# anshulahuja98/antidote

Hardware: AMD Instinct MI355X
Metric: materialized ops/sec + VC compares/sec (1/2/4/8 GPU), % of HBM roofline (higher is better)
Workload: dtype u64; 1 GPU; cfg2 counter_pn materialize: 10M keys x 64 ops/key, 8-DC clocks, random snapshot VCs; keys_per_gpu=10000000, keys_total=10000000, ops_per_key=64, n_dcs=8, r_jitter=U[-2000,2000], partitioning=vnode p = key mod 64, gpu = p mod G; no collective, parallelism=dp1

## Files before the change

antidote_amd/csrc/mat_counter_dense.hip:

```cpp
#include <atomic>
#include <cstdlib>
#include <vector>

#include "counter_scan.hpp"

namespace agn {
namespace {

constexpr uint32_t QL_S = 1024, QL_STRIDE = 32;

inline uint32_t counter_order(uint64_t n_req, uint32_t bulk) {
    return order_or(n_req < (1ull << 20) ? 1u : bulk);
}
constexpr uint32_t BULK_CHUNK = 64;
constexpr uint32_t BULK_CHUNK4 = 64;
constexpr bool Q2_FOUR_DEFAULT = true;
constexpr uint32_t BULK_CHUNK8 = 64;
constexpr uint64_t NARROW_WIDE_DIV = 1024;
constexpr bool EFF16_DEFAULT = true;
constexpr uint64_t EFF16_ESC_DIV = 1024;

struct DenseArgs {
    uint64_t n_req;
    uint64_t n_entries;
// ... 690 lines not shown
                                         uint32_t *__restrict__ o_count,
                                         uint32_t *__restrict__ o_flags,
                                         uint32_t *__restrict__ o_err,
                                         uint64_t *__restrict__ o_mask) {
    const int lane = lane_id();
    const uint64_t i = k.i;
    if (k.corrupt) {
        if (lane == 0) {
            o_flags[i] = AGN_F_ERR_CORRUPTED;
            o_err[i] = 0xffffffffu;
        }
        return;
    }
    if (lane < 4) {
        u64x2 v;
        v.x = r.ct_ign ? 0ull : s.ctA;
        v.y = r.ct_ign ? 0ull : s.ctB;
        reinterpret_cast<u64x2 *>(o_lastct + i * 8u)[lane] = v;
    }
    if (lane == 0) {
        o_value[i] = r.value;
        o_hole[i] = r.hole;
        o_count[i] = r.cnt;
        o_err[i] = r.err;
        o_flags[i] = r.fl;
        if (r.wm) o_mask[i] = r.mo;
    }
}

typedef long long i64x2 __attribute__((ext_vector_type(2)));
typedef unsigned int u32x2 __attribute__((ext_vector_type(2)));

__device__ __forceinline__ void q2_store2(uint64_t i0, const Q2Acc &s0, const Q2Acc &s1,
                                          const Q2Out &r0, const Q2Out &r1,
                                          int64_t *__restrict__ o_value,
                                          int64_t *__restrict__ o_hole,
                                          uint64_t *__restrict__ o_lastct,
                                          uint32_t *__restrict__ o_count,
                                          uint32_t *__restrict__ o_flags,
                                          uint32_t *__restrict__ o_err,
                                          uint64_t *__restrict__ o_mask) {
    const int lane = lane_id();
    if (lane < 8) {
        const bool hi = lane >= 4;
        const bool ign = hi ? r1.ct_ign : r0.ct_ign;
        u64x2 v;
        v.x = ign ? 0ull : (hi ? s1.ctA : s0.ctA);
        v.y = ign ? 0ull : (hi ? s1.ctB : s0.ctB);
        reinterpret_cast<u64x2 *>(o_lastct + i0 * 8u)[lane] = v;
    }
    if (lane == 0) {
        *reinterpret_cast<i64x2 *>(o_value + i0) = i64x2{r0.value, r1.value};
        *reinterpret_cast<i64x2 *>(o_hole + i0) = i64x2{r0.hole, r1.hole};
        *reinterpret_cast<u32x2 *>(o_count + i0) = u32x2{r0.cnt, r1.cnt};
        *reinterpret_cast<u32x2 *>(o_err + i0) = u32x2{r0.err, r1.err};
        *reinterpret_cast<u32x2 *>(o_flags + i0) = u32x2{r0.fl, r1.fl};
        if (r0.wm && r1.wm) {
            *reinterpret_cast<u64x2 *>(o_mask + i0) = u64x2{r0.mo, r1.mo};
        } else {
            if (r0.wm) o_mask[i0] = r0.mo;
            if (r1.wm) o_mask[i0 + 1u] = r1.mo;
        }
    }
}

struct Q2Params {
    DenseArgs a;
    MaskArgs mk;
    const uint64_t *keys, *key_off, *key_len;
    const uint8_t *key_type;
    const uint32_t *key_id0;
    const uint64_t *oc;
    const uint32_t *op_id;
    const int64_t *eff;
    const uint64_t *log_txid, *R, *sct;
    const uint8_t *sct_ignore;
    const uint64_t *req_txid;
    const int64_t *base_value;
    int64_t *o_value, *o_hole;
    uint64_t *o_lastct;
    uint32_t *o_count, *o_flags, *o_err, *list, *list_n;
};

template <class T>
__device__ __forceinline__ DenseArgs dense_of(const T &x) {
    return DenseArgs{x.n_req, x.n_entries, x.req_type, x.xcd, x.pair, x.qnt, x.hints, x.ql_cap};
}
template <class T>
__device__ __forceinline__ MaskArgs mask_of(const T &x) {
    return MaskArgs{x.key_mask, x.oc_mask, x.R_mask, x.sct_mask, x.o_mask};
}

__device__ __forceinline__ uint32_t put_lane(uint32_t v, int g, uint32_t old) {
    return lane_id() == g ? v : old;
}

struct Q2PackParams {
    DenseArgs a;
    MaskArgs mk;
    const void *args[20];
    const uint32_t *rows;
    const uint64_t *base;
    const uint8_t *ok;
};
static_assert(offsetof(Q2PackParams, rows) == offsetof(Q2Params, list),
              "Q2PackParams follows k_counter_quad2's parameter list");

__device__ __forceinline__ u32x4 q2_pack_thr(const Q2Key &k, const Q2Pack &p, bool &noR) {
    noR = ballot(k.rA < p.bq.x || k.rB < p.bq.y) != 0ull;
    const uint64_t dA = k.rA - p.bq.x, dB = k.rB - p.bq.y;
    const uint32_t tA = (dA >> 32) ? 0xFFFFFFFFu : (uint32_t)dA;
    const uint32_t tB = (dB >> 32) ? 0xFFFFFFFFu : (uint32_t)dB;
    u32x4 t;
    t.x = __builtin_amdgcn_update_dpp(0u, tA, 0x88, 0xF, 0xF, false);
    t.y = __builtin_amdgcn_update_dpp(0u, tB, 0x88, 0xF, 0xF, false);
    t.z = __builtin_amdgcn_update_dpp(0u, tA, 0xDD, 0xF, 0xF, false);
    t.w = __builtin_amdgcn_update_dpp(0u, tB, 0xDD, 0xF, 0xF, false);
    return t;
}

__device__ __forceinline__ void q2_pack_ct(const Q2Pack &p, u32x4 mx, Q2Acc &s) {
#pragma unroll
    for (int x = 2; x < AGN_WAVE; x <<= 1) {
        const uint32_t a = (uint32_t)__shfl_xor((int)mx.x, x, AGN_WAVE);
        const uint32_t b = (uint32_t)__shfl_xor((int)mx.y, x, AGN_WAVE);
        const uint32_t c = (uint32_t)__shfl_xor((int)mx.z, x, AGN_WAVE);
        const uint32_t d = (uint32_t)__shfl_xor((int)mx.w, x, AGN_WAVE);
        mx.x = a > mx.x ? a : mx.x;
        mx.y = b > mx.y ? b : mx.y;
        mx.z = c > mx.z ? c : mx.z;
        mx.w = d > mx.w ? d : mx.w;
    }
    const uint32_t g0 = __builtin_amdgcn_update_dpp(0u, mx.x, 0x50, 0xF, 0xF, false);
    const uint32_t g1 = __builtin_amdgcn_update_dpp(0u, mx.y, 0x50, 0xF, 0xF, false);
    const uint32_t g2 = __builtin_amdgcn_update_dpp(0u, mx.z, 0x50, 0xF, 0xF, false);
    const uint32_t g3 = __builtin_amdgcn_update_dpp(0u, mx.w, 0x50, 0xF, 0xF, false);
    const bool hi = (lane_id() & 1) != 0;
    s.ctA = s.cnt ? p.bq.x + (uint64_t)(hi ? g2 : g0) : 0ull;
    s.ctB = s.cnt ? p.bq.y + (uint64_t)(hi ? g3 : g1) : 0ull;
}

__device__ __forceinline__ void q2_serve_oc(const DenseArgs &a, uint64_t i) {
    const MaskArgs mk{};
    const auto &p = kparams<Q2Params>();
    const Q2Key k = q2_prologue<false, false>(a, mk, i, p.keys, p.key_off, p.key_len, p.key_type,
                                              p.key_id0, p.R, p.sct, p.sct_ignore, p.req_txid);
    Q2Acc s;
    s.ctA = k.eA;
    s.ctB = k.eB;
    if (a.n_entries != 0 && !k.corrupt)
        scan_key_q8<false, true, false, false>(p.oc, p.eff, nullptr, 0ull, k.off, k.n, a.n_entries,
                                               k.rA, k.rB, k.sA, k.sB, s.ctA, s.ctB, s.sum, s.cnt,
                                               s.first_excl, s.first_err, k.noR);
    const auto &pe = kparams<Q2Params>();
    q2_epilogue<false>(k, s, a.hints, pe.op_id, pe.base_value, pe.o_value, pe.o_hole, pe.o_lastct,
                       pe.o_count, pe.o_flags, pe.o_err, nullptr);
}

template <bool ANY_WARM, bool MSK, bool Q2_EFF, bool Q2_STORE, bool PACK = false>
__global__ __launch_bounds__(64, (ANY_WARM && !MSK) ? 6 : 1) void k_counter_quad2(
    DenseArgs a, MaskArgs mk, const uint64_t *__restrict__ keys,
    const uint64_t *__restrict__ key_off, const uint64_t *__restrict__ key_len,
    const uint8_t *__restrict__ key_type, const uint32_t *__restrict__ key_id0,
    const uint64_t *__restrict__ oc, const uint32_t *__restrict__ op_id,
    const int64_t *__restrict__ eff, const uint64_t *__restrict__ log_txid,
    const uint64_t *__restrict__ R, const uint64_t *__restrict__ sct,
    const uint8_t *__restrict__ sct_ignore, const uint64_t *__restrict__ req_txid,
    const int64_t *__restrict__ base_value, int64_t *__restrict__ o_value,
    int64_t *__restrict__ o_hole, uint64_t *__restrict__ o_lastct,
    uint32_t *__restrict__ o_count, uint32_t *__restrict__ o_flags,
    uint32_t *__restrict__ o_err, const uint32_t *__restrict__ pack_rows,
    const uint64_t *__restrict__ pack_base, const uint8_t *__restrict__ pack_ok) {
    static_assert(!PACK || (!ANY_WARM && !MSK && Q2_EFF && Q2_STORE),
                  "packed rows: the cold dense form only");
    const uint32_t blk = block_order(a.xcd, blockIdx.x, gridDim.x);
    const uint64_t i0 = uniform_u64((uint64_t)blk * 2u);
    if (i0 >= a.n_req) return;
    const bool two = i0 + 1u < a.n_req;
    const uint64_t i1 = two ? i0 + 1u : i0;
    Q2Pack pk0{}, pk1{};
    const Q2Key k0 = q2_prologue<ANY_WARM, MSK, PACK>(a, mk, i0, keys, key_off, key_len, key_type,
                                                      key_id0, R, sct, sct_ignore, req_txid,
                                                      pack_base, pack_ok, &pk0);
    const Q2Key k1 = q2_prologue<ANY_WARM, MSK, PACK>(a, mk, i1, keys, key_off, key_len, key_type,
                                                      key_id0, R, sct, sct_ignore, req_txid,
                                                      pack_base, pack_ok, &pk1);
    Q2Acc s0, s1;
    s0.ctA = k0.eA;
    s0.ctB = k0.eB;
    s1.ctA = k1.eA;
    s1.ctB = k1.eB;
    if constexpr (Q2_EFF || Q2_STORE) {
        const bool one = k0.n <= (uint64_t)AGN_WAVE && k1.n <= (uint64_t)AGN_WAVE;
        if (a.n_entries != 0 && one && (!MSK || (k0.uni && k1.uni)) &&
            (!PACK || (pk0.ok & pk1.ok) != 0u)) {
            const bool d0 = !k0.corrupt, d1 = !k1.corrupt;
            uint64_t in0 = 0, in1 = 0;
            int64_t ev0 = 0, ev1 = 0;
            u32x4 m0 = {0u, 0u, 0u, 0u}, m1 = {0u, 0u, 0u, 0u};
            if constexpr (PACK) {
                const uint32_t *const rows = kparams<Q2PackParams>().rows;
                const P8Rows c0 = p8_load_rows<true>(rows, k0.off, 0, a.n_entries);
                const P8Rows c1 = p8_load_rows<true>(rows, k1.off, 0, a.n_entries);
                const int64_t *const l_eff = (const int64_t *)kparams<Q2Params>().eff;
                const uint64_t *const l_R = (const uint64_t *)kparams<Q2Params>().R;
                __builtin_amdgcn_sched_barrier(0);
                bool nr0, nr1;
                const u32x4 th0 = q2_pack_thr(k0, pk0, nr0), th1 = q2_pack_thr(k1, pk1, nr1);
                Q2Acc t0 = s0, t1 = s1;
                in0 = p8_verdict(c0, 0, k0.n, th0, nr0, m0, t0.cnt, t0.first_excl);
                in0 = d0 ? in0 : 0ull;
                if (d0) s0 = t0;
                ev0 = q8_load_eff(l_eff, k0.off, 0, in0, reinterpret_cast<const int64_t *>(l_R + k0.i * 8u));
                in1 = p8_verdict(c1, 0, k1.n, th1, nr1, m1, t1.cnt, t1.first_excl);
                in1 = d1 ? in1 : 0ull;
                if (d1) s1 = t1;
                ev1 = q8_load_eff(l_eff, k1.off, 0, in1, reinterpret_cast<const int64_t *>(l_R + k1.i * 8u));
                __builtin_amdgcn_sched_barrier(0);
            } else if constexpr (Q2_EFF) {
                const Q8Rows c0 = q8_load_rows<true>(oc, k0.off, 0, a.n_entries);
                const Q8Rows c1 = q8_load_rows<true>(oc, k1.off, 0, a.n_entries);
                __builtin_amdgcn_sched_barrier(0);
                Q2Acc t0 = s0, t1 = s1;
                in0 = q2_verdict<ANY_WARM>(k0, c0, log_txid, a.n_entries, t0);
                in0 = d0 ? in0 : 0ull;
                if (d0) s0 = t0;
                ev0 = q8_load_eff(eff, k0.off, 0, in0, reinterpret_cast<const int64_t *>(R + k0.i * 8u));
                in1 = q2_verdict<ANY_WARM>(k1, c1, log_txid, a.n_entries, t1);
                in1 = d1 ? in1 : 0ull;
                if (d1) s1 = t1;
                ev1 = q8_load_eff(eff, k1.off, 0, in1, reinterpret_cast<const int64_t *>(R + k1.i * 8u));
                __builtin_amdgcn_sched_barrier(0);
            } else {
                const Q8Chunk c0 = q8_load<true, false>(oc, eff, k0.off, 0, a.n_entries);
                const Q8Chunk c1 = q8_load<true, false>(oc, eff, k1.off, 0, a.n_entries);
                __builtin_amdgcn_sched_barrier(0);
                if (d0) q2_fold<ANY_WARM>(k0, c0, 0, log_txid, a.n_entries, s0);
                if (d1) q2_fold<ANY_WARM>(k1, c1, 0, log_txid, a.n_entries, s1);
            }
            const auto &pr = kparams<Q2Params>();
            const uint32_t *const l_op_id = pr.op_id;
            const int64_t *const l_base = pr.base_value;
            int64_t *const l_value = pr.o_value, *const l_hole = pr.o_hole;
            uint64_t *const l_lastct = pr.o_lastct;
            uint32_t *const l_count = pr.o_count, *const l_flags = pr.o_flags, *const l_err = pr.o_err;
            if constexpr (PACK) {
                q2_pack_ct(pk0, m0, s0);
                q2_pack_ct(pk1, m1, s1);
            } else {
                q2_ctfold<MSK>(k0, s0);
                q2_ctfold<MSK>(k1, s1);
            }
            if constexpr (Q2_EFF) {
                __builtin_amdgcn_sched_barrier(0);
                q8_fold_eff(in0, ev0, 0, s0.sum, s0.first_err);
                q8_fold_eff(in1, ev1, 0, s1.sum, s1.first_err);
                __builtin_amdgcn_sched_barrier(0);
            }
            Q2Out r0{}, r1{};
            if (d0) r0 = q2_result<MSK>(k0, s0, a.hints, l_op_id, l_base, mk.o_mask != nullptr);
            if (two && d1) r1 = q2_result<MSK>(k1, s1, a.hints, l_op_id, l_base, mk.o_mask != nullptr);
            if (Q2_STORE && two && d0 && d1) {
                q2_store2(i0, s0, s1, r0, r1, l_value, l_hole, l_lastct, l_count, l_flags, l_err, mk.o_mask);
            } else {
                q2_store(k0, s0, r0, l_value, l_hole, l_lastct, l_count, l_flags, l_err, mk.o_mask);
                if (two) q2_store(k1, s1, r1, l_value, l_hole, l_lastct, l_count, l_flags, l_err, mk.o_mask);
            }
            return;
        }
    }
    if constexpr (PACK) {
#pragma nounroll
        for (uint32_t h = 0; h < (two ? 2u : 1u); ++h) q2_serve_oc(a, i0 + h);
        return;
    }
    if (a.n_entries != 0) {
        const Q8Chunk c0 = q8_load<true, false>(oc, eff, k0.off, 0, a.n_entries);
        const Q8Chunk c1 = q8_load<true, false>(oc, eff, k1.off, 0, a.n_entries);
        __builtin_amdgcn_sched_barrier(0);
        const bool d0 = !k0.corrupt && (!MSK || k0.uni), d1 = !k1.corrupt && (!MSK || k1.uni);
        if (d0) q2_fold<ANY_WARM>(k0, c0, 0, log_txid, a.n_entries, s0);
        if (d1) q2_fold<ANY_WARM>(k1, c1, 0, log_txid, a.n_entries, s1);
        if (d0) q2_rest<ANY_WARM>(k0, oc, eff, log_txid, a.n_entries, s0);
        if (d1) q2_rest<ANY_WARM>(k1, oc, eff, log_txid, a.n_entries, s1);
        if constexpr (MSK) {
            if (!k0.corrupt && !k0.uni)
                q2_msk<ANY_WARM>(k0, oc, mk.oc_mask, eff, log_txid, a.n_entries, s0);
            if (!k1.corrupt && !k1.uni)
                q2_msk<ANY_WARM>(k1, oc, mk.oc_mask, eff, log_txid, a.n_entries, s1);
        }
    }
    if constexpr (Q2_EFF || Q2_STORE) {
        const auto &pe = kparams<Q2Params>();
        q2_epilogue<MSK>(k0, s0, a.hints, pe.op_id, pe.base_value, pe.o_value, pe.o_hole, pe.o_lastct,
                         pe.o_count, pe.o_flags, pe.o_err, mk.o_mask);
        if (two)
            q2_epilogue<MSK>(k1, s1, a.hints, pe.op_id, pe.base_value, pe.o_value, pe.o_hole,
                             pe.o_lastct, pe.o_count, pe.o_flags, pe.o_err, mk.o_mask);
        return;
    }
    q2_epilogue<MSK>(k0, s0, a.hints, op_id, base_value, o_value, o_hole, o_lastct, o_count, o_flags, o_err,
                     mk.o_mask);
    if (two)
        q2_epilogue<MSK>(k1, s1, a.hints, op_id, base_value, o_value, o_hole, o_lastct, o_count, o_flags,
                         o_err, mk.o_mask);
}

__global__ __launch_bounds__(64) void k_counter_pack4(Q2PackParams) {
    const DenseArgs a = dense_of(kparams<Q2Params>().a);
    const uint32_t blk = block_order(a.xcd, blockIdx.x, gridDim.x);
    const uint64_t i0 = uniform_u64((uint64_t)blk * 4u);
    if (i0 >= a.n_req) return;
    const int lane = lane_id();
    if (i0 + 3u < a.n_req) {
        const auto &pm = kparams<Q2Params>();
        const uint64_t *const key_off = pm.key_off, *const key_len = pm.key_len;
        const uint32_t *const key_id0 = pm.key_id0;
        const uint8_t *const key_type = pm.key_type;
        const uint64_t *const R = pm.R;
        const auto &pq = *(const __attribute__((address_space(4))) Q2PackParams *)&pm;
        const uint64_t *const pbase = pq.base;
        const uint8_t *const pok = pq.ok;
        const int64_t *const bvp = pm.base_value;
        const u64x4 offv = ldc_u64x4(key_off + i0);
        const u64x4 lenv = ldc_u64x4(key_len ? key_len + i0 : key_off + i0);
        const u32x4 idv = ldc_u32x4(key_id0 ? key_id0 + i0
                                            : reinterpret_cast<const uint32_t *>(key_off + i0));
        const uint8_t *const ktp = key_type ? key_type : reinterpret_cast<const uint8_t *>(key_off);
        uint64_t off[5], ln[4];
        uint32_t id0[4];
        off[4] = uniform_u64(ldc(key_len ? key_off + i0 : key_off + i0 + 4u));
        uint32_t ktw = __builtin_amdgcn_readfirstlane(ldc(reinterpret_cast<const uint32_t *>(ktp) + (i0 >> 2)));
        uint32_t okw = __builtin_amdgcn_readfirstlane(ldc(reinterpret_cast<const uint32_t *>(pok) + (i0 >> 2)));
        const uint64_t slot = i0 * 8u + (uint64_t)p4_slot(lane);
        const uint64_t rv = R[slot], bv = pbase[slot];
        const uint64_t bvl = *(bvp ? reinterpret_cast<const uint64_t *>(bvp) + (i0 + (uint64_t)(lane & 3))
                                   : R + slot);
        const uint64_t reqbase = bvp ? bvl : 0ull;
#pragma unroll
        for (int g = 0; g < 4; ++g) {
            off[g] = uniform_u64(offv[g]);
            ln[g] = uniform_u64(lenv[g]);
            id0[g] = (uint32_t)__builtin_amdgcn_readfirstlane(idv[g]);
        }
        asm volatile("" : "+s"(off[0]), "+s"(off[1]), "+s"(off[2]), "+s"(off[3]), "+s"(off[4]),
                          "+s"(ln[0]), "+s"(ln[1]), "+s"(ln[2]), "+s"(ln[3]), "+s"(id0[0]),
                          "+s"(id0[1]), "+s"(id0[2]), "+s"(id0[3]), "+s"(ktw), "+s"(okw));
        const bool has_len = key_len != nullptr, has_id0 = key_id0 != nullptr;
        const uint32_t want = key_type != nullptr ? (a.req_type & 0xffu) * 0x01010101u : ktw;
        uint32_t n[4];
        uint32_t bad = (okw ^ 0x01010101u) | (a.n_entries == 0 ? 1u : 0u);
#pragma unroll
        for (int g = 0; g < 4; ++g) {
            const uint64_t n64 = has_len ? ln[g] : off[g + 1] - off[g];
            n[g] = (uint32_t)n64;
            id0[g] = has_id0 ? id0[g] : AGN_ID0_NONE;
            const uint32_t kdiff = ((ktw ^ want) >> (8 * g)) & 0xffu;
            bad |= (n64 > (uint64_t)AGN_WAVE ? 1u : 0u) | (n64 != 0 ? kdiff : 0u);
        }
        if (bad == 0u) {
            const uint32_t *const rows = kparams<Q2PackParams>().rows;
            P8Rows c[4];
#pragma unroll
            for (int g = 0; g < 4; ++g) c[g] = p8_load_rows<true>(rows, off[g], 0, a.n_entries);
            const int64_t *const l_eff = kparams<Q2Params>().eff;
            __builtin_amdgcn_sched_barrier(0);
            const uint64_t below = ballot(rv < bv);
            const uint64_t dl = rv - bv;
            const uint32_t t = (dl >> 32) ? 0xFFFFFFFFu : (uint32_t)dl;
            uint32_t v_off_lo = 0, v_off_hi = 0, v_n = 0, v_id0 = 0, v_cnt = 0, v_fx = 0, v_fe = 0,
                     v_sum_lo = 0, v_sum_hi = 0;
            uint32_t cg = 0;
            const int kg = lane >> 4;
            u32x4 mx[4];
            uint64_t in[4];
            int64_t ev[4];
#pragma unroll
            for (int g = 0; g < 4; ++g) {
                const u32x4 th = p4_thr(t, g);
                const bool noR = ((below >> (16 * g)) & 0xFFFFull) != 0ull;
                uint32_t cnt = 0;
                int64_t fx = -1;
                mx[g] = u32x4{0u, 0u, 0u, 0u};
                in[g] = p8_verdict(c[g], 0, (uint64_t)n[g], th, noR, mx[g], cnt, fx);
                ev[g] = q8_load_eff(l_eff, off[g], 0, in[g],
                                    reinterpret_cast<const int64_t *>(R + (i0 + (uint64_t)g) * 8u));
                __builtin_amdgcn_sched_barrier(0);
                cg = kg == g ? cnt : cg;
                v_cnt = put_lane(cnt, g, v_cnt);
                v_fx = put_lane((uint32_t)fx, g, v_fx);
                v_off_lo = put_lane((uint32_t)off[g], g, v_off_lo);
                v_off_hi = put_lane((uint32_t)(off[g] >> 32), g, v_off_hi);
                v_n = put_lane(n[g], g, v_n);
                v_id0 = put_lane(id0[g], g, v_id0);
            }
            __builtin_amdgcn_sched_barrier(0);
            const auto &pr = kparams<Q2Params>();
            const uint32_t *const l_op_id = pr.op_id;
            int64_t *const l_value = pr.o_value, *const l_hole = pr.o_hole;
            uint64_t *const l_lastct = pr.o_lastct;
            uint32_t *const l_count = pr.o_count, *const l_flags = pr.o_flags, *const l_err = pr.o_err;
            const uint64_t v_off = ((uint64_t)v_off_hi << 32) | v_off_lo;
            const int32_t fx = (int32_t)v_fx;
            const uint32_t pos = fx >= 0 ? (uint32_t)fx : v_n - 1u;
            const bool need = lane < 4 && v_id0 == AGN_ID0_NONE && v_n != 0u;
            const uint32_t *const ip = need ? l_op_id + (v_off + (uint64_t)pos)
                                            : reinterpret_cast<const uint32_t *>(R + slot);
            const uint32_t opid = *ip;
            const uint32_t md = p4_maxfold(mx);
            const uint64_t ct = cg ? bv + (uint64_t)md : 0ull;
            __builtin_amdgcn_sched_barrier(0);
#pragma unroll
            for (int g = 0; g < 4; ++g) {
                int64_t sum = 0, fe = -1;
                q8_fold_eff(in[g], ev[g], 0, sum, fe);
                const uint64_t total = (uint64_t)wave_sum_dpp(sum);
                v_fe = put_lane((uint32_t)fe, g, v_fe);
                v_sum_lo = put_lane((uint32_t)total, g, v_sum_lo);
                v_sum_hi = put_lane((uint32_t)(total >> 32), g, v_sum_hi);
            }
            __builtin_amdgcn_sched_barrier(0);
            const uint64_t idh = v_id0 != AGN_ID0_NONE ? (uint64_t)v_id0 + (uint64_t)pos : (uint64_t)opid;
            const int64_t hid = v_n ? (int64_t)idh : 0;
            const int32_t fe = (int32_t)v_fe;
            uint32_t fl = v_cnt ? AGN_F_NEWSS : AGN_F_CT_IGNORE;
            fl |= fe >= 0 ? AGN_F_ERR_UNEXPECTED : 0u;
            if ((lane & 2) == 0) l_lastct[slot] = ct;
            if (lane < 4) {
                const uint64_t i = i0 + (uint64_t)lane;
                l_value[i] = (int64_t)(reqbase + (((uint64_t)v_sum_hi << 32) | v_sum_lo));
                l_hole[i] = fx >= 0 ? hid - 1 : hid;
                l_count[i] = v_cnt;
                l_err[i] = fe >= 0 ? (uint32_t)(v_off + (uint64_t)fe) : 0xffffffffu;
                l_flags[i] = fl;
            }
            return;
        }
    }
    const uint64_t left = a.n_req - i0;
    const uint32_t m = left < 4u ? (uint32_t)left : 4u;
#pragma nounroll
    for (uint32_t h = 0; h < m; ++h) q2_serve_oc(a, i0 + h);
}

struct Q2Pack8Params {
    DenseArgs a;
    MaskArgs mk;
    const void *args[20];
    const uint32_t *rows;
    const uint64_t *base;
    const uint8_t *ok;
    const uint16_t *rows16;
    const uint8_t *narrow;
    const int16_t *eff16;
};
static_assert(offsetof(Q2Pack8Params, rows) == offsetof(Q2PackParams, rows) &&
                  offsetof(Q2Pack8Params, base) == offsetof(Q2PackParams, base),
              "Q2Pack8Params extends Q2PackParams");

template <bool E16>
__global__ __launch_bounds__(64) void k_counter_pack8(Q2Pack8Params) {
    const DenseArgs a = dense_of(kparams<Q2Params>().a);
    const uint32_t blk = block_order(a.xcd, blockIdx.x, gridDim.x);
    const uint64_t i0 = uniform_u64((uint64_t)blk * 8u);
    if (i0 >= a.n_req) return;
    const int lane = lane_id();
    if (i0 + 7u < a.n_req) {
        const auto &pm = kparams<Q2Params>();
        const uint64_t *const key_off = pm.key_off, *const key_len = pm.key_len;
        const uint32_t *const key_id0 = pm.key_id0;
        const uint8_t *const key_type = pm.key_type;
        const uint64_t *const R = pm.R;
        const int64_t *const bvp = pm.base_value;
        const auto &pq = *(const __attribute__((address_space(4))) Q2Pack8Params *)&pm;
        const uint64_t *const pbase = pq.base;
        const uint8_t *const pnar = pq.narrow;
        const bool has_len = key_len != nullptr, has_id0 = key_id0 != nullptr;
        const uint32_t m8 = (uint32_t)lane & 7u;
        const uint64_t *const op = key_off + i0 + (uint64_t)((!has_len && lane >= 8) ? 8u : m8);
        const uint64_t v_off = *op;
        const uint64_t v_lr = *(has_len ? key_len + i0 + m8 : op);
        const uint32_t v_ir = *(has_id0 ? key_id0 + i0 + m8 : reinterpret_cast<const uint32_t *>(op));
        const uint8_t *const ktp = key_type ? key_type : reinterpret_cast<const uint8_t *>(key_off);
        uint32_t ktw0 = __builtin_amdgcn_readfirstlane(ldc(reinterpret_cast<const uint32_t *>(ktp) + (i0 >> 2)));
        uint32_t ktw1 = __builtin_amdgcn_readfirstlane(ldc(reinterpret_cast<const uint32_t *>(ktp) + (i0 >> 2) + 1u));
        uint32_t nw0 = __builtin_amdgcn_readfirstlane(ldc(reinterpret_cast<const uint32_t *>(pnar) + (i0 >> 2)));
        uint32_t nw1 = __builtin_amdgcn_readfirstlane(ldc(reinterpret_cast<const uint32_t *>(pnar) + (i0 >> 2) + 1u));
        const uint64_t slot = i0 * 8u + (uint64_t)lane;
        const uint64_t rv = R[slot], bv = pbase[slot];
        const uint64_t bvl = *(bvp ? reinterpret_cast<const uint64_t *>(bvp) + (i0 + m8) : R + slot);
        const uint64_t reqbase = bvp ? bvl : 0ull;
        const uint64_t v_nx =
            ((uint64_t)__builtin_amdgcn_update_dpp(0u, (uint32_t)(v_off >> 32), 0x101, 0xF, 0xF, false) << 32) |
            __builtin_amdgcn_update_dpp(0u, (uint32_t)v_off, 0x101, 0xF, 0xF, false);
        const uint64_t v_n64 = has_len ? v_lr : v_nx - v_off;
        const uint32_t v_n = (uint32_t)v_n64;
        const uint32_t v_id0 = has_id0 ? v_ir : AGN_ID0_NONE;
        const uint32_t kt = (((lane & 4) ? ktw1 : ktw0) >> (8u * ((uint32_t)lane & 3u))) & 0xffu;
        const uint32_t want = key_type != nullptr ? (a.req_type & 0xffu) : kt;
        const bool lbad = lane < 8 && (v_n64 > (uint64_t)AGN_WAVE || (v_n64 != 0 && kt != want));
        const bool bad = ballot(lbad) != 0ull || nw0 != 0x01010101u || nw1 != 0x01010101u ||
                         a.n_entries == 0;
        if (!bad) {
            const uint16_t *const rows16 = kparams<Q2Pack8Params>().rows16;
            u32x4 c[8];
#pragma unroll
            for (int g = 0; g < 8; ++g)
                c[g] = n8_load_rows<true>(rows16, n8_readlane_u64(v_off, g), a.n_entries);
            const int64_t *const l_eff = kparams<Q2Params>().eff;
            uint32_t e16[E16 ? 8 : 1];
            if constexpr (E16) {
                const int16_t *const eff16 = kparams<Q2Pack8Params>().eff16;
#pragma unroll
                for (int g = 0; g < 8; ++g)
                    e16[g] = n8_load_eff16(eff16, n8_readlane_u64(v_off, g), a.n_entries);
            }
            __builtin_amdgcn_sched_barrier(0);
            const uint64_t below = ballot(rv < bv);
            const uint64_t dl = rv - bv;
            const uint32_t tp = n8_thr_pack(dl > 0xFFFFull ? 0xFFFFu : (uint32_t)dl);
            uint32_t v_cnt = 0, v_fx = 0, v_fe = E16 ? 0xFFFFFFFFu : 0u, v_inc = 0;
            uint32_t cg = 0;
            const int kg = lane >> 3;
            int64_t ev[E16 ? 1 : 8];
#pragma unroll
            for (int g = 0; g < 8; ++g) {
                const uint32_t th0 = __builtin_amdgcn_readlane(tp, 8 * g);
                const uint32_t th1 = __builtin_amdgcn_readlane(tp, 8 * g + 2);
                const uint32_t th2 = __builtin_amdgcn_readlane(tp, 8 * g + 4);
                const uint32_t th3 = __builtin_amdgcn_readlane(tp, 8 * g + 6);
                const uint32_t noR = (uint32_t)(below >> (8 * g)) & 0xFFu;
                const uint32_t n_g = __builtin_amdgcn_readlane(v_n, g);
                const uint64_t off_g = n8_readlane_u64(v_off, g);
                const bool valid = (uint32_t)lane < n_g;
                const bool ex = (noR | n8_excl(c[g], th0, th1, th2, th3)) != 0u;
                const bool mine = valid & !ex;
                const uint64_t exm = ballot(valid & ex);
                const uint32_t cnt = (uint32_t)__builtin_popcountll(ballot(mine));
                const uint32_t fx = exm ? (uint32_t)__builtin_ctzll(exm) : 0xFFFFFFFFu;
                if constexpr (!E16)
                    ev[g] = n8_load_eff(l_eff, off_g, mine,
                                        reinterpret_cast<const int64_t *>(R + (i0 + (uint64_t)g) * 8u));
                c[g].x = mine ? c[g].x : 0u;
                c[g].y = mine ? c[g].y : 0u;
                c[g].z = mine ? c[g].z : 0u;
                c[g].w = mine ? c[g].w : 0u;
                v_inc |= mine ? (1u << g) : 0u;
                __builtin_amdgcn_sched_barrier(0);
                cg = kg == g ? cnt : cg;
                v_cnt = put_lane(cnt, g, v_cnt);
                v_fx = put_lane(fx, g, v_fx);
            }
            __builtin_amdgcn_sched_barrier(0);
            const auto &pr = kparams<Q2Params>();
            const uint32_t *const l_op_id = pr.op_id;
            int64_t *const l_value = pr.o_value, *const l_hole = pr.o_hole;
            uint64_t *const l_lastct = pr.o_lastct;
            uint32_t *const l_count = pr.o_count, *const l_flags = pr.o_flags, *const l_err = pr.o_err;
            const int32_t fx = (int32_t)v_fx;
            const uint32_t pos = fx >= 0 ? (uint32_t)fx : v_n - 1u;
            const bool need = lane < 8 && v_id0 == AGN_ID0_NONE && v_n != 0u;
            const uint32_t *const ip = need ? l_op_id + (v_off + (uint64_t)pos)
                                            : reinterpret_cast<const uint32_t *>(R + slot);
            uint32_t opid = 0;
            if (!E16 || ballot(need) != 0ull) opid = *ip;
            uint32_t v_esc = 0, ks32 = 0;
            if constexpr (E16) {
                uint32_t sm[8];
#pragma unroll
                for (int g = 0; g < 8; ++g) {
                    const bool mine = ((v_inc >> g) & 1u) != 0u;
                    const bool esc = mine && e16[g] == 0x8000u;
                    v_esc |= esc ? (1u << g) : 0u;
                    sm[g] = (mine && !esc) ? (uint32_t)(int32_t)(int16_t)e16[g] : 0u;
                }
                ks32 = n8_sumfold32(sm);
                __builtin_amdgcn_sched_barrier(0);
            }
            const uint32_t md = n8_maxfold(c);
            const uint64_t ct = cg ? bv + (uint64_t)md : 0ull;
            __builtin_amdgcn_sched_barrier(0);
            uint64_t total;
            if constexpr (E16) {
                total = (uint64_t)(int64_t)(int32_t)__shfl((int)ks32, 8 * (int)m8, AGN_WAVE);
                if (ballot(v_esc != 0u) != 0ull) {
#pragma nounroll
                    for (int g = 0; g < 8; ++g) {
                        const bool esc = ((v_esc >> g) & 1u) != 0u;
                        if (ballot(esc) == 0ull) continue;
                        const uint64_t off_g = n8_readlane_u64(v_off, g);
                        int64_t x = 0;
                        if (esc) x = l_eff[off_g + (uint64_t)lane];
                        const bool badv = esc && x == AGN_EFFECT_INVALID;
                        const uint64_t be = ballot(badv);
                        const uint64_t xs = (uint64_t)wave_sum_dpp(badv ? 0 : x);
                        v_fe = put_lane(be ? (uint32_t)__builtin_ctzll(be) : 0xFFFFFFFFu, g, v_fe);
                        total += lane == g ? xs : 0ull;
                    }
                }
            } else {
                uint64_t sm[8];
#pragma unroll
                for (int g = 0; g < 8; ++g) {
                    const bool mine = ((v_inc >> g) & 1u) != 0u;
                    const bool badv = mine && ev[g] == AGN_EFFECT_INVALID;
                    const uint64_t be = ballot(badv);
                    v_fe = put_lane(be ? (uint32_t)__builtin_ctzll(be) : 0xFFFFFFFFu, g, v_fe);
                    sm[g] = (mine && !badv) ? (uint64_t)ev[g] : 0ull;
                }
                const uint64_t ks = n8_sumfold(sm);
                total =
                    ((uint64_t)(uint32_t)__shfl((int)(uint32_t)(ks >> 32), 8 * (int)m8, AGN_WAVE) << 32) |
                    (uint32_t)__shfl((int)(uint32_t)ks, 8 * (int)m8, AGN_WAVE);
            }
            __builtin_amdgcn_sched_barrier(0);
            const uint64_t idh = v_id0 != AGN_ID0_NONE ? (uint64_t)v_id0 + (uint64_t)pos : (uint64_t)opid;
            const int64_t hid = v_n ? (int64_t)idh : 0;
            const int32_t fe = (int32_t)v_fe;
            uint32_t fl = v_cnt ? AGN_F_NEWSS : AGN_F_CT_IGNORE;
            fl |= fe >= 0 ? AGN_F_ERR_UNEXPECTED : 0u;
            l_lastct[slot] = ct;
            if (lane < 8) {
                const uint64_t i = i0 + (uint64_t)lane;
                l_value[i] = (int64_t)(reqbase + total);
                l_hole[i] = fx >= 0 ? hid - 1 : hid;
                l_count[i] = v_cnt;
                l_err[i] = fe >= 0 ? (uint32_t)(v_off + (uint64_t)fe) : 0xffffffffu;
                l_flags[i] = fl;
            }
            return;
        }
    }
    const uint64_t left = a.n_req - i0;
    const uint32_t m = left < 8u ? (uint32_t)left : 8u;
#pragma nounroll
    for (uint32_t h = 0; h < m; ++h) q2_serve_oc(a, i0 + h);
}

template <bool ANY_WARM, bool KEYS, int KM>
__global__ __launch_bounds__(64) void k_counter_q8e(
    DenseArgs a, MaskArgs mk, const uint64_t *__restrict__ keys,
    const uint64_t *__restrict__ key_off, const uint64_t *__restrict__ key_len,
    const uint8_t *__restrict__ key_type, const uint32_t *__restrict__ key_id0,
    const uint64_t *__restrict__ oc, const uint32_t *__restrict__ op_id,
    const int64_t *__restrict__ eff, const uint64_t *__restrict__ log_txid,
    const uint64_t *__restrict__ R, const uint64_t *__restrict__ sct,
    const uint8_t *__restrict__ sct_ignore, const uint64_t *__restrict__ req_txid,
    const int64_t *__restrict__ base_value, int64_t *__restrict__ o_value,
    int64_t *__restrict__ o_hole, uint64_t *__restrict__ o_lastct,
    uint32_t *__restrict__ o_count, uint32_t *__restrict__ o_flags,
    uint32_t *__restrict__ o_err, uint32_t *__restrict__ list, uint32_t *__restrict__ list_n) {
    const uint32_t blk = block_order(a.xcd, blockIdx.x, gridDim.x);
    const uint64_t i = uniform_u64((uint64_t)blk);
    if (i >= a.n_req) return;
    Q2Key k;
    q2_meta(k, i, KEYS ? keys : nullptr, key_off, key_len, key_id0);
    auto mixed = [&](uint64_t kmw) {
        return !(mk.oc_mask == nullptr || (mk.key_mask && (kmw & 0xFFull)) || k.n == 0);
    };
    auto hand_on = [&]() {
        if (lane_id() == 0) {
            const uint32_t sl = (uint32_t)(i % QL_S);
            list[(uint64_t)sl * a.ql_cap + atomicAdd(list_n + sl * QL_STRIDE, 1u)] = (uint32_t)i;
        }
    };
    uint64_t kmw = 0;
    if constexpr (KM == 1) {
        kmw = key_word(mk, k.key, key_off);
        if (mixed(kmw)) {
            hand_on();
            return;
        }
    }
    const bool any = a.n_entries != 0;
    Q8Chunk c0{};
    if (any) c0 = q8_load<true, false>(oc, eff, k.off, 0, a.n_entries);
    Q2Raw x = q2_load<ANY_WARM, true>(k, a, mk, KM == 0, key_off, key_type, R, sct, sct_ignore,
                                      req_txid);
    __builtin_amdgcn_sched_barrier(0);
    q2_pin(x);
    if constexpr (KM == 0) kmw = x.kmw;
    q2_apply<ANY_WARM, true>(k, a, mk, x, kmw, key_type, sct, sct_ignore, req_txid);
    if (KM == 0 && mixed(kmw)) {
        hand_on();
        return;
    }
    Q2Acc s;
    s.ctA = k.eA;
    s.ctB = k.eB;
    if (any && !k.corrupt) {
        q2_fold<ANY_WARM>(k, c0, 0, log_txid, a.n_entries, s);
        q2_rest<ANY_WARM>(k, oc, eff, log_txid, a.n_entries, s);
    }
    q2_epilogue<true>(k, s, a.hints, op_id, base_value, o_value, o_hole, o_lastct, o_count, o_flags,
                      o_err, mk.o_mask);
}

template <bool ANY_WARM, bool KEYS>
__global__ __launch_bounds__(64) void k_counter_q8e2(Q2Params) {
    const DenseArgs a = dense_of(kparams<Q2Params>().a);
    const uint32_t blk = block_order(a.xcd, blockIdx.x, gridDim.x);
    const uint64_t i0 = uniform_u64((uint64_t)blk * 2u);
    if (i0 >= a.n_req) return;
    const bool two = i0 + 1u < a.n_req;
    const uint64_t i1 = two ? i0 + 1u : i0;
    Q2Key k0, k1;
    {
        const auto &p = kparams<Q2Params>();
        q2_meta(k0, i0, KEYS ? p.keys : nullptr, p.key_off, p.key_len, p.key_id0);
        q2_meta(k1, i1, KEYS ? p.keys : nullptr, p.key_off, p.key_len, p.key_id0);
    }
    const bool any = a.n_entries != 0;
    Q8Chunk c0{}, c1{};
    if (any) {
        const auto &p = kparams<Q2Params>();
        c0 = q8_load<true, false>(p.oc, p.eff, k0.off, 0, a.n_entries);
        c1 = q8_load<true, false>(p.oc, p.eff, k1.off, 0, a.n_entries);
    }
    __builtin_amdgcn_sched_barrier(0);
    const auto &ps = kparams<Q2Params>();
    const MaskArgs mk = mask_of(ps.mk);
    const uint64_t kmw0 = key_word(mk, k0.key, ps.key_off), kmw1 = key_word(mk, k1.key, ps.key_off);
    q2_side<ANY_WARM, true>(k0, a, mk, kmw0, ps.key_off, ps.key_type, ps.R, ps.sct,
                            ps.sct_ignore, ps.req_txid);
    q2_side<ANY_WARM, true>(k1, a, mk, kmw1, ps.key_off, ps.key_type, ps.R, ps.sct,
                            ps.sct_ignore, ps.req_txid);
    auto mixed = [&](const Q2Key &k, uint64_t kmw) {
        return !(mk.oc_mask == nullptr || (mk.key_mask && (kmw & 0xFFull)) || k.n == 0);
    };
    auto hand_on = [&](uint64_t i) {
        if (lane_id() == 0) {
            const auto &p = kparams<Q2Params>();
            const uint32_t sl = (uint32_t)(i % QL_S);
            p.list[(uint64_t)sl * a.ql_cap + atomicAdd(p.list_n + sl * QL_STRIDE, 1u)] = (uint32_t)i;
        }
    };
    const bool m0 = mixed(k0, kmw0), m1 = two && mixed(k1, kmw1);
    if (m0) hand_on(i0);
    if (m1) hand_on(i1);
    Q2Acc s0, s1;
    s0.ctA = k0.eA;
    s0.ctB = k0.eB;
    s1.ctA = k1.eA;
    s1.ctB = k1.eB;
    const bool d0 = any && !k0.corrupt && !m0, d1 = two && any && !k1.corrupt && !m1;
    {
        const auto &p = kparams<Q2Params>();
        if (d0) q2_fold<ANY_WARM>(k0, c0, 0, p.log_txid, a.n_entries, s0);
        if (d1) q2_fold<ANY_WARM>(k1, c1, 0, p.log_txid, a.n_entries, s1);
        if (d0) q2_rest<ANY_WARM>(k0, p.oc, p.eff, p.log_txid, a.n_entries, s0);
        if (d1) q2_rest<ANY_WARM>(k1, p.oc, p.eff, p.log_txid, a.n_entries, s1);
    }
    const auto &pe = kparams<Q2Params>();
    if (!m0)
        q2_epilogue<true>(k0, s0, a.hints, pe.op_id, pe.base_value, pe.o_value, pe.o_hole,
                          pe.o_lastct, pe.o_count, pe.o_flags, pe.o_err, pe.mk.o_mask);
    if (two && !m1)
        q2_epilogue<true>(k1, s1, a.hints, pe.op_id, pe.base_value, pe.o_value, pe.o_hole,
                          pe.o_lastct, pe.o_count, pe.o_flags, pe.o_err, pe.mk.o_mask);
}

template <bool ANY_WARM, bool KEYS>
__global__ __launch_bounds__(64) void k_counter_q8m(
    DenseArgs a, MaskArgs mk, const uint64_t *__restrict__ keys,
    const uint64_t *__restrict__ key_off, const uint64_t *__restrict__ key_len,
    const uint8_t *__restrict__ key_type, const uint32_t *__restrict__ key_id0,
    const uint64_t *__restrict__ oc, const uint32_t *__restrict__ op_id,
    const int64_t *__restrict__ eff, const uint64_t *__restrict__ log_txid,
    const uint64_t *__restrict__ R, const uint64_t *__restrict__ sct,
    const uint8_t *__restrict__ sct_ignore, const uint64_t *__restrict__ req_txid,
    const int64_t *__restrict__ base_value, int64_t *__restrict__ o_value,
    int64_t *__restrict__ o_hole, uint64_t *__restrict__ o_lastct,
    uint32_t *__restrict__ o_count, uint32_t *__restrict__ o_flags,
    uint32_t *__restrict__ o_err, const uint32_t *__restrict__ list,
    const uint32_t *__restrict__ list_n) {
    const uint32_t sl = blockIdx.x % QL_S, per = gridDim.x / QL_S;
    const uint32_t cnt = __builtin_amdgcn_readfirstlane(list_n[sl * QL_STRIDE]);
    for (uint32_t j = blockIdx.x / QL_S; j < cnt; j += per) {
        const uint64_t i = __builtin_amdgcn_readfirstlane(list[(uint64_t)sl * a.ql_cap + j]);
        const Q2Key k = q2_prologue<ANY_WARM, true>(a, mk, i, KEYS ? keys : nullptr, key_off,
                                                    key_len, key_type, key_id0, R, sct, sct_ignore,
                                                    req_txid);
        Q2Acc s;
        s.ctA = k.eA;
        s.ctB = k.eB;
        if (a.n_entries != 0 && !k.corrupt)
            q2_msk<ANY_WARM>(k, oc, mk.oc_mask, eff, log_txid, a.n_entries, s);
        q2_epilogue<true>(k, s, a.hints, op_id, base_value, o_value, o_hole, o_lastct, o_count,
                          o_flags, o_err, mk.o_mask);
    }
}

MaskArgs mask_args(const agn_log &log, const agn_read &req, const agn_result &out) {
    MaskArgs m;
    m.key_mask = log.oc_mask ? log.key_mask : nullptr;
    m.oc_mask = log.oc_mask;
    m.R_mask = req.R_mask;
    m.sct_mask = req.sct ? req.sct_mask : nullptr;
    m.o_mask = out.lastct_mask;
    return m;
}

inline bool sparse_batch(const agn_log &log, const agn_read &req, const agn_result &out) {
    return log.oc_mask || req.R_mask || (req.sct && req.sct_mask) || out.lastct_mask;
}

int launch_quad2(const agn_log &log, const agn_read &req, const agn_result &out, hipStream_t st) {
    DenseArgs a{req.n_req, log.n_entries, req.req_type, counter_order(req.n_req, BULK_CHUNK), 0u, 1u,
                req.hints};
    const MaskArgs mk = mask_args(log, req, out);
    const uint64_t nb = (req.n_req + 1) / 2;
    if (nb > 0x7fffffffull) return fail(AGN_EINVAL, "batch too large: %llu requests",
                                        (unsigned long long)req.n_req);
    PackIdx pk{};
#define AGN_Q2L_(W, M, E, S, ...)                                                               \
    hipLaunchKernelGGL((k_counter_quad2<W, M, E, S, ##__VA_ARGS__>), dim3((unsigned)nb),        \
                       dim3(64), 0, st, a,                                                      \
                       mk, req.keys, log.key_off, log.key_len, log.key_type, id0_index(log),    \
                       log.oc, log.op_id, log.eff, log.txid, req.R, req.sct, req.sct_ignore,    \
                       req.txid, req.base_value, out.value, out.hole, out.lastct, out.count,    \
                       out.flags, out.err_pos, pk.rows, pk.base, pk.ok)
#define AGN_Q2L(W, M)                                                                           \
    do {                                                                                        \
        if (q2e && q2s) AGN_Q2L_(W, M, true, true);                                             \
        else if (q2e) AGN_Q2L_(W, M, true, false);                                              \
        else if (q2s) AGN_Q2L_(W, M, false, true);                                              \
        else AGN_Q2L_(W, M, false, false);                                                      \
    } while (0)
    const bool msk = sparse_batch(log, req, out);
    const bool dflt = !req.sct && !msk;
    const char *ev = AGN_KNOB("AGN_Q2_EFF"), *sv = AGN_KNOB("AGN_Q2_STORE");
    const bool q2e = (ev && (ev[0] == '0' || ev[0] == '1')) ? ev[0] == '1' : dflt;
    const uintptr_t a16 = (uintptr_t)out.value | (uintptr_t)out.hole | (uintptr_t)out.lastct |
                          (uintptr_t)mk.o_mask;
    const uintptr_t a8 = (uintptr_t)out.count | (uintptr_t)out.flags | (uintptr_t)out.err_pos;
    const bool q2s = ((sv && (sv[0] == '0' || sv[0] == '1')) ? sv[0] == '1' : dflt) &&
                     (a16 & 15u) == 0 && (a8 & 7u) == 0;
    const char *pv = AGN_KNOB("AGN_Q2_PACK");
    const bool pack = dflt && q2e && q2s && log.n_entries != 0 && !(pv && pv[0] == '0') &&
                      pack_lookup(log, &pk);
    const char *fv = AGN_KNOB("AGN_Q2_FOUR");
    const bool four = pack && !req.keys && log.n_entries / 64u <= log.n_keys &&
                      ((fv && (fv[0] == '0' || fv[0] == '1')) ? fv[0] == '1' : Q2_FOUR_DEFAULT);
    const char *nv = AGN_KNOB("AGN_Q2_NARROW");
    const bool eight = four && pk.rows16 && pk.narrow &&
                       ((nv && (nv[0] == '0' || nv[0] == '1'))
                            ? nv[0] == '1'
                            : pk.n_wide * NARROW_WIDE_DIV <= log.n_keys);
    const char *xv = AGN_KNOB("AGN_Q2_EFF16");
    const bool e16 = eight && pk.eff16 && log.eff == pk.eff_src &&
                     ((xv && (xv[0] == '0' || xv[0] == '1'))
                          ? xv[0] == '1'
                          : EFF16_DEFAULT && pk.n_esc * EFF16_ESC_DIV <= log.n_entries);
    if (eight) {
        a.xcd = counter_order(req.n_req, BULK_CHUNK8);
        const Q2Pack8Params p{a, mk,
                              {req.keys, log.key_off, log.key_len, log.key_type, id0_index(log),
                               log.oc, log.op_id, log.eff, log.txid, req.R, req.sct, req.sct_ignore,
                               req.txid, req.base_value, out.value, out.hole, out.lastct, out.count,
                               out.flags, out.err_pos},
                              pk.rows, pk.base, pk.ok, pk.rows16, pk.narrow, pk.eff16};
        const dim3 grid((unsigned)((req.n_req + 7) / 8));
        if (e16) hipLaunchKernelGGL(k_counter_pack8<true>, grid, dim3(64), 0, st, p);
        else hipLaunchKernelGGL(k_counter_pack8<false>, grid, dim3(64), 0, st, p);
    } else if (four) {
        a.xcd = counter_order(req.n_req, BULK_CHUNK4);
        const Q2PackParams p{a, mk,
                             {req.keys, log.key_off, log.key_len, log.key_type, id0_index(log),
                              log.oc, log.op_id, log.eff, log.txid, req.R, req.sct, req.sct_ignore,
                              req.txid, req.base_value, out.value, out.hole, out.lastct, out.count,
                              out.flags, out.err_pos},
                             pk.rows, pk.base, pk.ok};
        hipLaunchKernelGGL(k_counter_pack4, dim3((unsigned)((req.n_req + 3) / 4)), dim3(64), 0, st, p);
    } else if (pack) {
        AGN_Q2L_(false, false, true, true, true);
    } else if (req.sct) {
        if (msk) AGN_Q2L(true, true);
        else AGN_Q2L(true, false);
    } else {
        if (msk) AGN_Q2L(false, true);
        else AGN_Q2L(false, false);
    }
#undef AGN_Q2L
#undef AGN_Q2L_
    AGN_HIP(hipGetLastError());
    return AGN_OK;
}

inline bool early_chunk() {
    const char *v = AGN_KNOB("AGN_COUNTER_EARLY");
    return !(v && v[0] == '0');
}

int launch_q8e(const agn_log &log, const agn_read &req, const agn_result &out, hipStream_t st) {
    DenseArgs a{req.n_req, log.n_entries, req.req_type, counter_order(req.n_req, BULK_CHUNK), 0u, 1u,
                req.hints};
    const MaskArgs mk = mask_args(log, req, out);
    if (req.n_req > 0x7fffffffull) return fail(AGN_EINVAL, "batch too large: %llu requests",
                                               (unsigned long long)req.n_req);
    const char *kv = AGN_KNOB("AGN_Q8E_KM");
    const bool km0 = !(kv && kv[0] == '1');
    a.ql_cap = (uint32_t)((req.n_req + QL_S - 1) / QL_S);
    const size_t hdr = (size_t)QL_S * QL_STRIDE;
    uint32_t *lst = nullptr;
    AGN_HIP(pool_malloc(&lst, (hdr + (size_t)QL_S * a.ql_cap) * sizeof(uint32_t), st));
    int rc = AGN_OK;
    if (hipMemsetAsync(lst, 0, hdr * sizeof(uint32_t), st) != hipSuccess)
        rc = fail(AGN_EHIP, "counter q8e: list reset");
#define AGN_ARGS                                                                                \
    a, mk, req.keys, log.key_off, log.key_len, log.key_type, id0_index(log), log.oc, log.op_id,  \
        log.eff, log.txid, req.R, req.sct, req.sct_ignore, req.txid, req.base_value, out.value,  \
        out.hole, out.lastct, out.count, out.flags, out.err_pos, lst + hdr, lst
#define AGN_Q8E_(W, K, KM)                                                                      \
    hipLaunchKernelGGL((k_counter_q8e<W, K, KM>), dim3((unsigned)req.n_req), dim3(64), 0, st,   \
                       AGN_ARGS)
#define AGN_Q8E(W, K)                                                                           \
    do {                                                                                        \
        if (km0) AGN_Q8E_(W, K, 0);                                                             \
        else AGN_Q8E_(W, K, 1);                                                                 \
    } while (0)
    const unsigned mb = QL_S * 16u;
#define AGN_Q8M(W, K)                                                                           \
    hipLaunchKernelGGL((k_counter_q8m<W, K>), dim3(mb), dim3(64), 0, st, AGN_ARGS)
    const char *tv = AGN_KNOB("AGN_Q8E_TWO");
    const bool two = !(tv && tv[0] == '0');
    const bool two_cold = two && !(tv && tv[0] == '1');
    const unsigned nb2 = (unsigned)((req.n_req + 1) / 2);
#define AGN_Q8E2(W, K)                                                                          \
    hipLaunchKernelGGL((k_counter_q8e2<W, K>), dim3(nb2), dim3(64), 0, st, Q2Params{AGN_ARGS})
    if (rc == AGN_OK) {
        if (req.sct && two) {
            if (req.keys) { AGN_Q8E2(true, true); AGN_Q8M(true, true); }
            else { AGN_Q8E2(true, false); AGN_Q8M(true, false); }
        } else if (two_cold) {
            if (req.keys) { AGN_Q8E2(false, true); AGN_Q8M(false, true); }
            else { AGN_Q8E2(false, false); AGN_Q8M(false, false); }
        } else if (req.sct) {
            if (req.keys) { AGN_Q8E(true, true); AGN_Q8M(true, true); }
            else { AGN_Q8E(true, false); AGN_Q8M(true, false); }
        } else {
            if (req.keys) { AGN_Q8E(false, true); AGN_Q8M(false, true); }
            else { AGN_Q8E(false, false); AGN_Q8M(false, false); }
        }
        if (hipGetLastError() != hipSuccess) rc = fail(AGN_EHIP, "counter q8e: launch");
    }
#undef AGN_Q8E2
#undef AGN_Q8M
#undef AGN_Q8E
#undef AGN_Q8E_
#undef AGN_ARGS
    const hipError_t ef = hipFreeAsync(lst, st);
    if (rc == AGN_OK && ef != hipSuccess) rc = fail(AGN_EHIP, "hipFreeAsync: %s", hipGetErrorString(ef));
    return rc;
}

inline uint32_t pair_chunks() {
    const char *v = AGN_KNOB("AGN_COUNTER_PAIR");
    return (v && v[0] == '0') ? 0u : 1u;
}

constexpr int kMaxDev = 64;
std::atomic<int> g_rows_choice[kMaxDev];

template <int D>
constexpr int default_variant() { return D == 8 ? ROWS_QUAD : ROWS_VGPR; }

inline int cur_dev() {
    int d = 0;
    (void)hipGetDevice(&d);
    return d >= 0 && d < kMaxDev ? d : 0;
}

inline int forced_variant() {
    const char *v = AGN_KNOB("AGN_COUNTER_VARIANT");
    if (v && v[0] >= '0' && v[0] <= '3') return v[0] - '0';
    v = AGN_KNOB("AGN_COUNTER_GLDS");
    if (v && (v[0] == '0' || v[0] == '1')) return v[0] - '0';
    return -1;
}

inline int tuned_variant() {
    return g_rows_choice[cur_dev()].load(std::memory_order_relaxed) - 1;
}

template <int D>
int counter_variant() {
    const int f = forced_variant();
    if (f >= 0) return f;
    const int t = tuned_variant();
    return t >= 0 ? t : default_variant<D>();
}

template <int D, int WPB, int VAR, bool KEYS, bool MSK>
int launch_key_k(const agn_log &log, const agn_read &req, const agn_result &out, hipStream_t st) {
    const char *qv = AGN_KNOB("AGN_COUNTER_QUAD_NT");
    DenseArgs a{req.n_req, log.n_entries, req.req_type, counter_order(req.n_req, BULK_CHUNK), pair_chunks(),
                (qv && qv[0] >= '0' && qv[0] <= '3') ? (uint32_t)(qv[0] - '0') : 1u};
    const MaskArgs mk = mask_args(log, req, out);
    const uint64_t nb = (req.n_req + WPB - 1) / WPB;
    if (nb > 0x7fffffffull) return fail(AGN_EINVAL, "batch too large: %llu requests",
                                        (unsigned long long)req.n_req);
    if (req.sct)
        hipLaunchKernelGGL((k_counter_key<D, true, WPB, VAR, KEYS, MSK>), dim3((unsigned)nb),
                           dim3(64 * WPB), 0, st, a, mk, req.keys, log.key_off, log.key_len,
                           log.key_type, id0_index(log), log.oc, log.op_id, log.eff, log.txid,
                           req.R, req.sct, req.sct_ignore, req.txid, req.base_value, out.value,
                           out.hole, out.lastct, out.count, out.flags, out.err_pos);
    else
        hipLaunchKernelGGL((k_counter_key<D, false, WPB, VAR, KEYS, MSK>), dim3((unsigned)nb),
                           dim3(64 * WPB), 0, st, a, mk, req.keys, log.key_off, log.key_len,
                           log.key_type, id0_index(log), log.oc, log.op_id, log.eff, log.txid,
                           req.R, req.sct, req.sct_ignore, req.txid, req.base_value, out.value,
                           out.hole, out.lastct, out.count, out.flags, out.err_pos);
    AGN_HIP(hipGetLastError());
    return AGN_OK;
}

// ... 471 lines not shown
```

Measured before the change: 281.6 billion ops/s.

## Extend packed 8-key narrow counter kernel to warm snapshot requests with sct

Adds a WARM variant of the 8-keys-per-wave packed kernel that also reads the snapshot-commit vector and ignore flags, computes a second threshold mask, and filters ops already included in the snapshot. Requests carrying sct (warm path) previously fell through to the slower generic quad2 kernel; the new variant routes them through the compact rows16/eff16 packed layout. It adds extra per-slot loads and ballots, plus a new scalar fallback for tail keys.

```diff
diff --git a/antidote_amd/csrc/mat_counter_dense.hip b/antidote_amd/csrc/mat_counter_dense.hip
--- a/antidote_amd/csrc/mat_counter_dense.hip
+++ b/antidote_amd/csrc/mat_counter_dense.hip
@@ -866,6 +866,29 @@
         scan_key_q8<false, true, false, false>(p.oc, p.eff, nullptr, 0ull, k.off, k.n, a.n_entries,
                                                k.rA, k.rB, k.sA, k.sB, s.ctA, s.ctB, s.sum, s.cnt,
                                                s.first_excl, s.first_err, k.noR);
+    const auto &pe = kparams<Q2Params>();
+    q2_epilogue<false>(k, s, a.hints, pe.op_id, pe.base_value, pe.o_value, pe.o_hole, pe.o_lastct,
+                       pe.o_count, pe.o_flags, pe.o_err, nullptr);
+}
+
+__device__ __forceinline__ void q2_serve_oc_warm(const DenseArgs &a, uint64_t i) {
+    const MaskArgs mk{};
+    const auto &p = kparams<Q2Params>();
+    const Q2Key k = q2_prologue<true, false>(a, mk, i, p.keys, p.key_off, p.key_len, p.key_type,
+                                             p.key_id0, p.R, p.sct, p.sct_ignore, nullptr);
+    Q2Acc s;
+    s.ctA = k.eA;
+    s.ctB = k.eB;
+    if (a.n_entries != 0 && !k.corrupt) {
+        if (!k.sct_ign)
+            scan_key_q8<true, true, false, false>(p.oc, p.eff, nullptr, 0ull, k.off, k.n,
+                                                  a.n_entries, k.rA, k.rB, k.sA, k.sB, s.ctA, s.ctB,
+                                                  s.sum, s.cnt, s.first_excl, s.first_err, k.noR);
+        else
+            scan_key_q8<false, true, false, false>(p.oc, p.eff, nullptr, 0ull, k.off, k.n,
+                                                   a.n_entries, k.rA, k.rB, k.sA, k.sB, s.ctA, s.ctB,
+                                                   s.sum, s.cnt, s.first_excl, s.first_err, k.noR);
+    }
     const auto &pe = kparams<Q2Params>();
     q2_epilogue<false>(k, s, a.hints, pe.op_id, pe.base_value, pe.o_value, pe.o_hole, pe.o_lastct,
                        pe.o_count, pe.o_flags, pe.o_err, nullptr);
@@ -1172,8 +1195,9 @@
                   offsetof(Q2Pack8Params, base) == offsetof(Q2PackParams, base),
               "Q2Pack8Params extends Q2PackParams");
 
-template <bool E16>
+template <bool E16, bool WARM>
 __global__ __launch_bounds__(64) void k_counter_pack8(Q2Pack8Params) {
+    static_assert(!WARM || E16, "the warm form reads the effect tier");
     const DenseArgs a = dense_of(kparams<Q2Params>().a);
     const uint32_t blk = block_order(a.xcd, blockIdx.x, gridDim.x);
     const uint64_t i0 = uniform_u64((uint64_t)blk * 8u);
@@ -1204,6 +1228,18 @@
         const uint64_t rv = R[slot], bv = pbase[slot];
         const uint64_t bvl = *(bvp ? reinterpret_cast<const uint64_t *>(bvp) + (i0 + m8) : R + slot);
         const uint64_t reqbase = bvp ? bvl : 0ull;
+        uint64_t sv = 0;
+        uint32_t igw0 = 0, igw1 = 0;
+        if constexpr (WARM) {
+            const uint64_t *const sct = pm.sct;
+            const uint8_t *const sig = pm.sct_ignore;
+            sv = sct[slot];
+            const uint8_t *const sgp = sig ? sig : reinterpret_cast<const uint8_t *>(key_off);
+            igw0 = __builtin_amdgcn_readfirstlane(ldc(reinterpret_cast<const uint32_t *>(sgp) + (i0 >> 2)));
+            igw1 = __builtin_amdgcn_readfirstlane(ldc(reinterpret_cast<const uint32_t *>(sgp) + (i0 >> 2) + 1u));
+            igw0 = sig ? igw0 : 0u;
+            igw1 = sig ? igw1 : 0u;
+        }
         const uint64_t v_nx =
             ((uint64_t)__builtin_amdgcn_update_dpp(0u, (uint32_t)(v_off >> 32), 0x101, 0xF, 0xF, false) << 32) |
             __builtin_amdgcn_update_dpp(0u, (uint32_t)v_off, 0x101, 0xF, 0xF, false);
@@ -1233,6 +1269,13 @@
             const uint64_t below = ballot(rv < bv);
             const uint64_t dl = rv - bv;
             const uint32_t tp = n8_thr_pack(dl > 0xFFFFull ? 0xFFFFu : (uint32_t)dl);
+            uint64_t belowS = 0;
+            uint32_t ts = 0;
+            if constexpr (WARM) {
+                belowS = ballot(sv < bv);
+                const uint64_t ds = sv - bv;
+                ts = n8_thr_pack(ds > 0xFFFFull ? 0xFFFFu : (uint32_t)ds);
+            }
             uint32_t v_cnt = 0, v_fx = 0, v_fe = E16 ? 0xFFFFFFFFu : 0u, v_inc = 0;
             uint32_t cg = 0;
             const int kg = lane >> 3;
@@ -1248,8 +1291,18 @@
                 const uint64_t off_g = n8_readlane_u64(v_off, g);
                 const bool valid = (uint32_t)lane < n_g;
                 const bool ex = (noR | n8_excl(c[g], th0, th1, th2, th3)) != 0u;
-                const bool mine = valid & !ex;
-                const uint64_t exm = ballot(valid & ex);
+                bool nip = true;
+                if constexpr (WARM) {
+                    const uint32_t ts0 = __builtin_amdgcn_readlane(ts, 8 * g);
+                    const uint32_t ts1 = __builtin_amdgcn_readlane(ts, 8 * g + 2);
+                    const uint32_t ts2 = __builtin_amdgcn_readlane(ts, 8 * g + 4);
+                    const uint32_t ts3 = __builtin_amdgcn_readlane(ts, 8 * g + 6);
+                    const uint32_t ign_g = (((g & 4) ? igw1 : igw0) >> (8 * (g & 3))) & 0xFFu;
+                    const uint32_t noS = (uint32_t)(belowS >> (8 * g)) & 0xFFu;
+                    nip = (ign_g | noS | n8_excl(c[g], ts0, ts1, ts2, ts3)) != 0u;
+                }
+                const bool mine = valid & nip & !ex;
+                const uint64_t exm = ballot(valid & nip & ex);
                 const uint32_t cnt = (uint32_t)__builtin_popcountll(ballot(mine));
                 const uint32_t fx = exm ? (uint32_t)__builtin_ctzll(exm) : 0xFFFFFFFFu;
                 if constexpr (!E16)
@@ -1292,7 +1345,14 @@
                 __builtin_amdgcn_sched_barrier(0);
             }
             const uint32_t md = n8_maxfold(c);
-            const uint64_t ct = cg ? bv + (uint64_t)md : 0ull;
+            uint64_t ct = cg ? bv + (uint64_t)md : 0ull;
+            uint32_t ign_r = 0;
+            if constexpr (WARM) {
+                const uint32_t ign_l = (((kg & 4) ? igw1 : igw0) >> (8u * ((uint32_t)kg & 3u))) & 0xFFu;
+                const uint64_t seed = ign_l ? 0ull : sv;
+                ct = seed > ct ? seed : ct;
+                ign_r = (((lane & 4) ? igw1 : igw0) >> (8u * ((uint32_t)lane & 3u))) & 0xFFu;
+            }
             __builtin_amdgcn_sched_barrier(0);
             uint64_t total;
             if constexpr (E16) {
@@ -1331,7 +1391,7 @@
             const uint64_t idh = v_id0 != AGN_ID0_NONE ? (uint64_t)v_id0 + (uint64_t)pos : (uint64_t)opid;
             const int64_t hid = v_n ? (int64_t)idh : 0;
             const int32_t fe = (int32_t)v_fe;
-            uint32_t fl = v_cnt ? AGN_F_NEWSS : AGN_F_CT_IGNORE;
+            uint32_t fl = v_cnt ? AGN_F_NEWSS : ((!WARM || ign_r) ? AGN_F_CT_IGNORE : 0u);
             fl |= fe >= 0 ? AGN_F_ERR_UNEXPECTED : 0u;
             l_lastct[slot] = ct;
             if (lane < 8) {
@@ -1347,8 +1407,13 @@
     }
     const uint64_t left = a.n_req - i0;
     const uint32_t m = left < 8u ? (uint32_t)left : 8u;
+    if constexpr (WARM) {
 #pragma nounroll
-    for (uint32_t h = 0; h < m; ++h) q2_serve_oc(a, i0 + h);
+        for (uint32_t h = 0; h < m; ++h) q2_serve_oc_warm(a, i0 + h);
+    } else {
+#pragma nounroll
+        for (uint32_t h = 0; h < m; ++h) q2_serve_oc(a, i0 + h);
+    }
 }
 
 template <bool ANY_WARM, bool KEYS, int KM>
@@ -1566,7 +1631,25 @@
                      ((xv && (xv[0] == '0' || xv[0] == '1'))
                           ? xv[0] == '1'
                           : EFF16_DEFAULT && pk.n_esc * EFF16_ESC_DIV <= log.n_entries);
-    if (eight) {
+    const char *wv = AGN_KNOB("AGN_Q2_WARM8");
+    PackIdx wk{};
+    const bool warm8 =
+        req.sct && !msk && !req.keys && log.n_entries != 0 && (!req.txid || !log.txid) &&
+        !(wv && wv[0] == '0') && log.n_entries / 64u <= log.n_keys && pack_lookup(log, &wk) &&
+        wk.rows16 && wk.narrow && wk.eff16 && log.eff == wk.eff_src &&
+        ((wv && wv[0] == '1') || (wk.n_wide * NARROW_WIDE_DIV <= log.n_keys && EFF16_DEFAULT &&
+                                  wk.n_esc * EFF16_ESC_DIV <= log.n_entries));
+    if (warm8) {
+        a.xcd = counter_order(req.n_req, BULK_CHUNK8);
+        const Q2Pack8Params p{a, mk,
+                              {req.keys, log.key_off, log.key_len, log.key_type, id0_index(log),
+                               log.oc, log.op_id, log.eff, log.txid, req.R, req.sct, req.sct_ignore,
+                               req.txid, req.base_value, out.value, out.hole, out.lastct, out.count,
+                               out.flags, out.err_pos},
+                              wk.rows, wk.base, wk.ok, wk.rows16, wk.narrow, wk.eff16};
+        hipLaunchKernelGGL((k_counter_pack8<true, true>), dim3((unsigned)((req.n_req + 7) / 8)),
+                           dim3(64), 0, st, p);
+    } else if (eight) {
         a.xcd = counter_order(req.n_req, BULK_CHUNK8);
         const Q2Pack8Params p{a, mk,
                               {req.keys, log.key_off, log.key_len, log.key_type, id0_index(log),
@@ -1575,8 +1658,8 @@
                                out.flags, out.err_pos},
                               pk.rows, pk.base, pk.ok, pk.rows16, pk.narrow, pk.eff16};
         const dim3 grid((unsigned)((req.n_req + 7) / 8));
-        if (e16) hipLaunchKernelGGL(k_counter_pack8<true>, grid, dim3(64), 0, st, p);
-        else hipLaunchKernelGGL(k_counter_pack8<false>, grid, dim3(64), 0, st, p);
+        if (e16) hipLaunchKernelGGL((k_counter_pack8<true, false>), grid, dim3(64), 0, st, p);
+        else hipLaunchKernelGGL((k_counter_pack8<false, false>), grid, dim3(64), 0, st, p);
     } else if (four) {
         a.xcd = counter_order(req.n_req, BULK_CHUNK4);
         const Q2PackParams p{a, mk,
```

New measurement: 264.3 billion ops/s. 6.1% lower.
